# jerinphilip/whisper.tflite

Measured on AMD Instinct MI355X. Metric: audio-sec/s (RTF) whisper-tiny 30s clips batch=32 at 1/2/4/8 MI355X, higher is better.
Workload: dtype f32 (operands as two fp16 planes, f16 MFMA, f32 accumulate); 1 GPU; whisper-tiny batch=32x30s synthetic mel U(-1,1.5), fp32, random-init weights (BASELINE.json configs[1]); mel resident in HBM -> token ids on host; clips_per_gpu=32, global_batch=32, decoder_positions=30, argmax_steps=27, parallelism=clip-parallel dp1, one RCCL all_gather of id records per 8 batches, pipelined=True, batches_in_flight=10, decoder=2 consecutive steps' batches share one decoder chain (dec_pair, dec_group), last_batches_announced=2, priming_batches=1

## Files before the change

### include/wt_debug.h

```cpp
#ifndef WT_DEBUG_H_
#define WT_DEBUG_H_
#include "wt_capi.h"
#ifdef __cplusplus
extern "C" {
#endif
int wt_dbg_gemm(wt_engine* h, int M, int N, int K, const float* A, const float* W, const float* bias,
                const float* R, const float* pos, int pos_period, int epi, float* C);
int wt_dbg_gemm_planes(wt_engine* h, int M, int N, int K, const float* A, const float* W, const float* bias,
                       const float* R, const float* pos, int pos_period, int epi, int planes_out, int iters, float* C,
                       float* avg_ms, int n_cu );
int wt_dbg_set_forced_ids(wt_engine* h, const int64_t* ids, int clips);
int wt_dbg_set_plane_gemm_mode(int mode);
int wt_dbg_gemm_planes_ln(wt_engine* h, int M, int K, const float* A, const float* W, const float* bias, const float* R,
                          const float* pos, int pos_period, int epi, const float* ln_g, const float* ln_b, int n_cu,
                          float* C, float* ln_out, float* ln_y32, int* fused);
int wt_dbg_encoder_attention_planes(wt_engine* h, int batch, int T, int heads, const float* qkv, int iters, float* out,
                                    float* avg_ms);
int wt_dbg_gemm_bench(wt_engine* h, int M, int N, int K, int epi, int variant, int iters, float* avg_ms);
int wt_dbg_interference(wt_engine* h, const float* d_mel, int batch, int n_enc, int chain_len, int blocks,
                        float* enc_ms, float* chain_ms);
int wt_dbg_concurrency(wt_engine* h, const float* d_mel, int batch, int n_dec, int n_enc, float* dec_ms,
                       float* enc_ms);
int wt_dbg_dec_gemm_bench(wt_engine* h, int kind, int B, int N, int K, int rows, int iters, float* avg_us);
int wt_dbg_dec_gemm(wt_engine* h, int mode, int B, int N, int K, const float* X, const float* W,
                    const float* bias, const float* R, float* Y, int64_t* argmax_out);
int wt_dbg_dec_ln_gemm(wt_engine* h, int B, int N, int K, const float* xin, const int64_t* ids, int pos,
                       const float* tok_emb, const float* pos_emb, int n_vocab, int n_pos,
// ... 179 lines not shown
```

### whisper.tflite_amd/__init__.py

```python
from __future__ import annotations

import ctypes
import enum
import os
import types
from ctypes import (POINTER, byref, c_char_p, c_float, c_int, c_int32, c_int64, c_long, c_size_t,
                    c_uint64, c_void_p)

import numpy as np

_HERE = os.path.dirname(os.path.abspath(__file__))
LIB_PATH = os.environ.get("WT_LIB_PATH") or os.path.join(_HERE, "lib", "libwhisper-tflite.so")

WT_OK = 0
WT_MAX_IDS = 32
WT_PIPELINE_DEPTH = 24
WT_LANGUAGE_AUTO = -1
CHUNK_SAMPLES = 480000
STATUS_NAMES = {0: "WT_OK", 1: "WT_ERR_INVALID_ARG", 2: "WT_ERR_IO", 3: "WT_ERR_FORMAT",
                4: "WT_ERR_UNSUPPORTED", 5: "WT_ERR_DEVICE", 6: "WT_ERR_BUFFER"}

CAPI_SYMBOLS = [
    "wt_device_alloc", "wt_device_free", "wt_device_upload", "wt_device_download", "wt_device_synchronize",
    "wt_engine_create", "wt_engine_destroy", "wt_last_error", "wt_engine_dims",
# ... 4 lines not shown
    "wt_encdec_tokens_full_batch", "wt_encdec_tokens_full_batch_dev", "wt_transcribe_tokens_full_batch_dev",
    "wt_last_segments", "wt_last_segment_text", "wt_vocab_segments", "wt_vocab_seek_step", "wt_last_windows",
    "wt_transcribe_long_batch", "wt_last_file_text", "wt_last_window_files",
    "wt_vocab_split_words", "wt_vocab_merge_punctuation", "wt_dtw_path",
    "wt_engine_set_alignment_heads", "wt_last_words", "wt_last_word_text",
    "wt_last_scores", "wt_last_token_logprobs", "wt_last_segment_scores", "wt_last_decode_info", "wt_last_best_of",
    "wt_language_count", "wt_detect_language_batch", "wt_detect_language_batch_dev", "wt_detect_language_pcm", "wt_last_languages",
    "wt_last_timings", "wt_last_beam_scores", "wt_last_kernel_stats", "wt_decode_text", "wt_language_id", "wt_lang_code", "wt_wav_read_legacy",
    "wt_vocab_info", "wt_filters", "wt_write_synthetic_weights", "wt_write_synthetic_vocab",
    "wt_vocab_open", "wt_vocab_close", "wt_vocab_get_info", "wt_vocab_get_filters", "wt_vocab_size", "wt_vocab_token",
    "wt_vocab_decode", "wt_log_mel_spectrogram", "wt_convert_tflite", "wt_shutdown",
]
DEBUG_SYMBOLS = [
    "wt_dbg_cross_absorbed", "wt_dbg_cross_absorbed_bf16", "wt_dbg_gemm_planes_ln", "wt_dbg_gemm", "wt_dbg_gemm_bench", "wt_dbg_dec_gemm_bench", "wt_dbg_dec_gemm", "wt_dbg_dec_ln_gemm", "wt_dbg_layernorm", "wt_dbg_encoder_attention",
    "wt_dbg_cross_attention", "wt_dbg_self_attention", "wt_dbg_interference", "wt_dbg_concurrency",
    "wt_dbg_gemm_planes", "wt_dbg_set_plane_gemm_mode", "wt_dbg_set_forced_ids", "wt_dbg_dec_gemm_bf16", "wt_dbg_dec_ln_gemm_bf16",
    "wt_dbg_self_attention_bf16", "wt_dbg_cross_attention_bf16", "wt_dbg_encoder_attention_planes", "wt_dbg_gemm_bf16", "wt_dbg_gemm_bf16_ln", "wt_dbg_encoder_attention_bf16",
    "wt_dbg_beam_topk", "wt_dbg_beam_step", "wt_dbg_beam_reorder", "wt_dbg_beam_finalize",
    "wt_dbg_beam_full_step", "wt_dbg_beam_full_finalize",
    "wt_dbg_dec_gemm_ksplit", "wt_dbg_dec_ln_gemm_rows", "wt_dbg_dec_logits", "wt_dbg_select_token",
    "wt_dbg_cross_absorbed_chain", "wt_dbg_absorbed_query_matrix", "wt_dbg_language_head", "wt_dbg_self_attention_long",
    "wt_dbg_self_attention_prefill", "wt_dbg_self_attention_long_gather",
    "wt_dbg_self_attention_long_ragged", "wt_dbg_self_attention_prefill_ragged", "wt_dbg_dec_ln_gemm_ragged", "wt_dbg_ragged_cap",
    "wt_dbg_timestamp_select", "wt_dbg_token_scores", "wt_dbg_sample_select", "wt_dbg_suppress_logits",
    "wt_dbg_sample_select_group", "wt_dbg_best_of_begin", "wt_dbg_best_of_pick",
    "wt_dbg_frontend_dims", "wt_dbg_frontend_stages", "wt_dbg_log_clipmax", "wt_dbg_mel_normalize", "wt_dbg_mel_transpose",
    "wt_dbg_pcm_to_planes",
    "wt_dbg_gemm_addressed", "wt_dbg_plane_gemm_plan", "wt_dbg_gemm_ln_fused", "wt_dbg_layernorm_planes", "wt_dbg_f32_to_planes", "wt_dbg_encoder_attention_at",
    "wt_dbg_encoder_scales", "wt_dbg_f16_scale_for", "wt_dbg_gemm_planes_scaled",
    "wt_dbg_cross_attention_records", "wt_dbg_cross_attention_records_bf16", "wt_dbg_cross_combine", "wt_dbg_cross_combine_bf16",
    "wt_dbg_align_scores", "wt_dbg_align_matrix", "wt_dbg_align_dtw", "wt_dbg_last_alignment", "wt_dbg_set_alignment",
# ... 102 lines not shown
        L.wt_write_synthetic_weights.argtypes = [c_char_p, c_char_p, c_uint64]
        L.wt_write_synthetic_vocab.argtypes = [c_char_p, c_int]
        L.wt_vocab_open.argtypes = [c_char_p, c_int, POINTER(c_void_p)]
        L.wt_vocab_close.argtypes = [c_void_p]
        L.wt_vocab_close.restype = None
        L.wt_vocab_get_info.argtypes = [c_void_p, ip32]
        L.wt_vocab_get_filters.argtypes = [c_void_p, fp, c_size_t, ip32, ip32]
        L.wt_vocab_size.argtypes = [c_void_p]
        L.wt_vocab_token.argtypes = [c_void_p, c_int, c_char_p, c_size_t, POINTER(c_size_t)]
        L.wt_vocab_decode.argtypes = [c_void_p, ip64, c_int, c_int, c_char_p, c_size_t, POINTER(c_size_t)]
        L.wt_log_mel_spectrogram.argtypes = [fp, c_int, fp, c_int, c_int, c_int, fp, c_size_t, POINTER(c_int)]
        L.wt_convert_tflite.argtypes = [c_char_p, c_char_p]
        L.wt_dbg_gemm.argtypes = [c_void_p, c_int, c_int, c_int, fp, fp, fp, fp, fp, c_int, c_int, fp]
        L.wt_dbg_gemm_planes.argtypes = [c_void_p, c_int, c_int, c_int, fp, fp, fp, fp, fp, c_int, c_int, c_int, c_int, fp,
                                         POINTER(c_float), c_int]
        L.wt_dbg_encoder_attention_planes.argtypes = [c_void_p, c_int, c_int, c_int, fp, c_int, fp, POINTER(c_float)]
        L.wt_dbg_cross_absorbed.argtypes = [c_void_p, c_int, c_int, c_int, c_int, c_int, fp, fp, fp, fp, fp, c_int, POINTER(c_float)]
        L.wt_dbg_cross_absorbed_bf16.argtypes = L.wt_dbg_cross_absorbed.argtypes
        L.wt_dbg_cross_absorbed_chain.argtypes = [c_void_p, c_int, c_int, c_int, c_int, c_int, c_int, c_int, c_int, POINTER(fp),
                                                  fp, fp, fp, c_int, c_int, c_int, fp, fp]
        L.wt_dbg_absorbed_query_matrix.argtypes = [c_int, c_int, fp, fp, fp, fp, fp]
        L.wt_dbg_gemm_planes_ln.argtypes = [c_void_p, c_int, c_int, fp, fp, fp, fp, fp, c_int, c_int, fp, fp, c_int, fp, fp, fp,
                                            POINTER(c_int)]
        L.wt_dbg_gemm_bf16.argtypes = [c_void_p, c_int, c_int, c_int, fp, fp, fp, fp, fp, c_int, c_int, c_int, c_int, fp,
                                       POINTER(c_float)]
        L.wt_dbg_encoder_attention_bf16.argtypes = [c_void_p, c_int, c_int, c_int, fp, c_int, fp, POINTER(c_float)]
        L.wt_dbg_gemm_bf16_ln.argtypes = [c_void_p, c_int, c_int, c_int, fp, fp, fp, fp, fp, fp, fp, fp, fp, POINTER(c_int)]
        L.wt_dbg_gemm_bench.argtypes = [c_void_p, c_int, c_int, c_int, c_int, c_int, c_int, POINTER(c_float)]
        L.wt_dbg_dec_gemm_bench.argtypes = [c_void_p, c_int, c_int, c_int, c_int, c_int, c_int, POINTER(c_float)]
        L.wt_dbg_dec_gemm.argtypes = [c_void_p, c_int, c_int, c_int, c_int, fp, fp, fp, fp, fp, ip64]
# ... 719 lines not shown

    def dbg_gemm_planes(self, A, W, bias=None, R=None, pos=None, epi=1, planes_out=False, iters=0, n_cu=0):
        A, W = _f32(A), _f32(W)
        M, K = A.shape
        N = W.shape[0]
        C = np.zeros((M, N), np.float32)
        bias = _f32(bias) if bias is not None else np.zeros(N, np.float32)
        R = _f32(R) if R is not None else None
        pos = _f32(pos) if pos is not None else None
        ms = c_float(0)
        self._check(lib().wt_dbg_gemm_planes(self._h, M, N, K, _fp(A), _fp(W), _fp(bias), _fp(R), _fp(pos),
                                             pos.shape[0] if pos is not None else 0, epi, int(planes_out), iters, _fp(C),
                                             byref(ms), int(n_cu)))
        return (C, ms.value) if iters > 0 else C

    def dbg_gemm_planes_ln(self, A, W, bias, ln_g, ln_b, R=None, pos=None, epi=5, n_cu=0, want_y32=True):
        A, W = _f32(A), _f32(W)
        M, K = A.shape
        assert W.shape[0] == 384
        C = np.zeros((M, 384), np.float32)
        ln = np.zeros((M, 384), np.float32)
        y32 = np.zeros((M, 384), np.float32) if want_y32 else None
        R = _f32(R) if R is not None else None
        pos = _f32(pos) if pos is not None else None
        fused = ctypes.c_int(0)
        self._check(lib().wt_dbg_gemm_planes_ln(self._h, M, K, _fp(A), _fp(W), _fp(_f32(bias)), _fp(R), _fp(pos),
                                                pos.shape[0] if pos is not None else 0, epi, _fp(_f32(ln_g)), _fp(_f32(ln_b)),
                                                int(n_cu), _fp(C), _fp(ln), _fp(y32) if y32 is not None else None, byref(fused)))
        return C, ln, y32, bool(fused.value)

# ... 832 lines not shown
```

### whisper.tflite_amd/csrc/capi_debug.cpp

```cpp
#include "wt_debug.h"

#include <hip/hip_runtime.h>

#include <algorithm>
#include <array>
#include <cmath>
#include <cstdio>
#include <cstdlib>
#include <cstring>
#include <limits>
#include <memory>
#include <vector>

#include "capi_internal.h"
#include "kernels.h"

namespace {
template <class T>
struct DevArr {
  T* p = nullptr;
  size_t n = 0;
  explicit DevArr(size_t n_, const T* host = nullptr) : n(n_) {
    hipchk(hipMalloc(reinterpret_cast<void**>(&p), std::max<size_t>(n, 1) * sizeof(T)), "hipMalloc");
    if (host && n) hipchk(hipMemcpy(p, host, n * sizeof(T), hipMemcpyHostToDevice), "H2D");
// ... 197 lines not shown
int wt_dbg_gemm_planes(wt_engine* h, int M, int N, int K, const float* A, const float* W, const float* bias,
                       const float* R, const float* pos, int pos_period, int epi, int planes_out, int iters, float* C,
                       float* avg_ms, int n_cu) {
  if (!h || !A || !W || !C || N % 128 || K % 32 || M < 1 || n_cu < 0) return WT_ERR_INVALID_ARG;
  return guarded(h, [&] {
    const float sa = wt::f16_scale_for(max_abs(A, size_t(M) * K)), sw = wt::f16_scale_for(max_abs(W, size_t(N) * K));
    const DevPlanes dA(A, size_t(M) * K, sa);
    const DevArr<unsigned short> dW(weight_planes(W, N, K, sw));
    DevArr<float> dB(N, bias), dC(size_t(M) * N, R), dP(pos ? size_t(pos_period) * N : 0, pos);
    const float out_bound = max_abs(A, size_t(M) * K) * max_abs(W, size_t(N) * K) * float(K) + (bias ? max_abs(bias, N) : 0.0f);
    const float so = wt::f16_scale_for(out_bound);
    DevPlanes dO(nullptr, size_t(M) * N, 1.0f);
    wt::PlaneGemmArgs g;
    dense_gemm_args(g, M, N, K, dB.p, dC.p, dP.p, pos_period);
    g.A = dA.ptr(); g.a_plane = dA.plane; g.W = dW.p; g.a_scale = sa; g.w_scale = sw; g.n_cu = n_cu;
    if (planes_out) { g.P = dO.ptr(); g.p_plane = dO.plane; g.out_scale[0] = so; }
    hipStream_t st = h->impl->stream();
    wt::launch_gemm_planes(g, epi, st);
    h->impl->sync();
    if (planes_out) dO.to_host(C, size_t(M) * N, so); else dC.to_host(C, size_t(M) * N);
    if (avg_ms && iters > 0) *avg_ms = time_launches(st, 3, iters, [&] { wt::launch_gemm_planes(g, epi, st); });
  });
}

int wt_dbg_set_forced_ids(wt_engine* h, const int64_t* ids, int clips) {
  if (!h || clips < 0 || clips > 4096 || (clips && !ids)) return WT_ERR_INVALID_ARG;
  return guarded(h, [&] {
    h->impl->forced_ids.assign(ids, ids + size_t(clips) * 32);
    for (long long v : h->impl->forced_ids)
      if (v < 0) throw wt::Error(wt::kErrInvalidArg, "forced ids must be token ids");
  });
}

int wt_dbg_set_plane_gemm_mode(int mode) {
  if (mode < 0 || mode > 4) return WT_ERR_INVALID_ARG;
  wt::set_plane_gemm_mode(mode);
  return WT_OK;
}

int wt_dbg_gemm_planes_ln(wt_engine* h, int M, int K, const float* A, const float* W, const float* bias, const float* R,
                          const float* pos, int pos_period, int epi, const float* ln_g, const float* ln_b, int n_cu,
                          float* C, float* ln_out, float* ln_y32, int* fused) {
  const int N = 384;
  if (!h || !A || !W || !C || !ln_g || !ln_b || !ln_out || !fused || K % 32 || M < 1 || n_cu < 0) return WT_ERR_INVALID_ARG;
  return guarded(h, [&] {
    const float sa = wt::f16_scale_for(max_abs(A, size_t(M) * K)), sw = wt::f16_scale_for(max_abs(W, size_t(N) * K));
    const DevPlanes dA(A, size_t(M) * K, sa);
    const DevArr<unsigned short> dW(weight_planes(W, N, K, sw));
    DevArr<float> dB(N, bias), dC(size_t(M) * N, R), dP(pos ? size_t(pos_period) * N : 0, pos), dG(N, ln_g), dS(N, ln_b),
        dY(size_t(M) * N);
    DevArr<int> dF(1);
    hipStream_t st = h->impl->stream();
// ... 1441 lines not shown
    g.kv_batch = kv_batch; g.kv_heads = kv_heads; g.kv_dmodel = kv_dmodel;
    g.M = M; g.N = N; g.K = K; g.n_cu = n_cu;
    DevArr<float> dC(out_format == 0 ? size_t(c_len) : 0, static_cast<const float*>(out));
    DevArr<unsigned short> dO(out_format == 1 ? 2 * size_t(c_len) : out_format == 2 ? size_t(c_len) : 0,
                              static_cast<const unsigned short*>(out));
    if (out_format == 0) {
      g.C = dC.p + c_off; g.R = g.C;
    } else {
      g.P = dO.p + c_off; g.p_plane = c_len; g.seg = seg;
      if (out_format == 1) g.out_scale[0] = out_scale[0], g.out_scale[1] = out_scale[1], g.out_scale[2] = out_scale[2];
    }
    if (kind == 1) {
      const float sa = wt::f16_scale_for(max_abs(A, size_t(a_len))), sw = wt::f16_scale_for(max_abs(W, size_t(N) * K));
      const DevPlanes dA(A, size_t(a_len), sa);
      const DevArr<unsigned short> dW(weight_planes(W, N, K, sw));
      g.A = dA.ptr(); g.a_plane = dA.plane; g.W = dW.p; g.a_scale = sa; g.w_scale = sw;
      wt::launch_gemm_planes(g, epi, st);
      h->impl->sync();
    } else {
      const DevBf16 dA(A, size_t(a_len)), dW(W, size_t(N) * K);
      g.A = dA.ptr(); g.W = dW.ptr();
      wt::launch_gemm_bf16_planes(g, epi, st);
      h->impl->sync();
    }
    if (out_format == 0) dC.to_host(static_cast<float*>(out)); else dO.to_host(static_cast<unsigned short*>(out));
  });
}

int wt_dbg_plane_gemm_plan(int family, int M, int N, int K, int epi, int planes_out, int ln, int n_cu, int c_rpb, int ldc,
                           int32_t plan[4]) {
  if (!plan || family < 0 || family > 1 || M < 1 || N < 1 || K < 1 || n_cu < 0) return WT_ERR_INVALID_ARG;
// ... 106 lines not shown
                              int guard_rows, void* out) {
  const bool epi_ok = planes_out ? (epi == wt::kEpiBias || epi == (wt::kEpiBias | wt::kEpiGelu))
                                 : (epi == wt::kEpiBias || epi == (wt::kEpiBias | wt::kEpiGelu) || epi == (wt::kEpiBias | wt::kEpiResidual));
  if (!h || !A || !W || !bias || !out || !out_scale || !epi_ok || M < 1 || N < 128 || N % 128 || K < 32 || K % 32 || n_cu < 0 ||
      guard_rows < 0 || seg < 0) {
    return WT_ERR_INVALID_ARG;
  }
  return guarded(h, [&] {
    const size_t cells = size_t(M + guard_rows) * N;
    const DevPlanes dA(A, size_t(M) * K, a_scale);
    const DevArr<unsigned short> dW(weight_planes(W, N, K, w_scale));
    DevArr<float> dB(N, bias), dC(planes_out ? 0 : cells, static_cast<const float*>(out));
    DevArr<unsigned short> dO(planes_out ? 2 * cells : 0, static_cast<const unsigned short*>(out));
    wt::PlaneGemmArgs g;
    dense_gemm_args(g, M, N, K, dB.p, planes_out ? nullptr : dC.p, nullptr, 0);
    g.A = dA.ptr(); g.a_plane = dA.plane; g.W = dW.p; g.a_scale = a_scale; g.w_scale = w_scale; g.n_cu = n_cu;
    if (planes_out) {
      g.P = dO.p; g.p_plane = long(cells); g.seg = seg;
      g.out_scale[0] = out_scale[0]; g.out_scale[1] = out_scale[1]; g.out_scale[2] = out_scale[2];
    }
    wt::launch_gemm_planes(g, epi, h->impl->stream());
    h->impl->sync();
    if (planes_out) dO.to_host(static_cast<unsigned short*>(out)); else dC.to_host(static_cast<float*>(out));
  });
}

int wt_dbg_encoder_attention_at(wt_engine* h, int kind, int variant, int batch, int T, int heads, int guard_rows,
                                const float* qkv, const float scales[4], void* out) {
  if (!h || !qkv || !out || kind < 0 || kind > 2 || guard_rows < 0 || batch < 0 || T < 0 || heads < 0 || (kind == 1 && !scales)) {
    return WT_ERR_INVALID_ARG;
  }
// ... 143 lines not shown
```

### whisper.tflite_amd/csrc/engine.cpp

```cpp
#include "engine_internal.h"

#include <fcntl.h>
#include <sys/mman.h>
#include <sys/stat.h>
#include <unistd.h>

#include <chrono>
#include <cmath>
#include <complex>
#include <cstdio>
#include <cstdlib>
#include <cstring>
#include <stdexcept>

#include "kernels.h"

namespace wt {

namespace {
size_t round_up(size_t v, size_t m) { return (v + m - 1) / m * m; }
}


std::vector<unsigned short> tile_weights_f16(const float* W, int N, int K, float* scale) {
// ... 678 lines not shown
    const int prio = dp && dp[0] == 'l' ? prio_lo : prio_hi;
    for (auto& ds : dstream_) HIPCHK(hipStreamCreateWithPriority(&ds, hipStreamNonBlocking, prio));
  }
  pick_decoder_streams();
  for (auto& e : ev_) HIPCHK(hipEventCreate(&e));
  for (Slot& sl : slots_) {
    for (hipEvent_t* e : {&sl.enc_begin, &sl.enc_mid, &sl.enc_done, &sl.dec_begin, &sl.dec_done}) {
      HIPCHK(hipEventCreate(e));
    }
    sl.h_ids = pinned<long long>(4096 * 32);
    sl.h_n = pinned<int>(4096);
    sl.h_flag = pinned<int>(1);
    *sl.h_flag = 0;
    HIPCHK(hipMalloc(reinterpret_cast<void**>(&sl.d_flag), sizeof(int)));
  }
}

Engine::Engine(const std::string& model_prefix, const std::string& vocab_path, bool multilingual,
               int device_id, bool monolith, const std::string& weights_path)
    : device_(device_id), monolith_(monolith), multilingual_(multilingual) {
  read_vocab_file(vocab_path, multilingual, &filters_, &vocab_);
  if (monolith) language = 0;
  open_device();
  try {
    create_streams();
    upload_weights(weights_path.empty() ? model_prefix + ".wtw" : weights_path);
    if (vocab_.n_vocab != dims_.n_vocab && verbose) {
      std::fprintf(stderr, "[wt] note: vocab file n_vocab %d != model n_vocab %d\n", vocab_.n_vocab,
                   dims_.n_vocab);
    }
// ... 14 lines not shown
    build_frontend_tables();
  } catch (...) {
    release();
    throw;
  }
}

Engine::~Engine() { release(); }

void Engine::release() noexcept {
  (void)hipSetDevice(device_);
  for (hipStream_t st : {stream_full_, stream_masked_})
    if (st) (void)hipStreamSynchronize(st);
  for (auto& ds : dstream_)
    if (ds) (void)hipStreamSynchronize(ds);
  for (auto& g : graphs_) (void)hipGraphExecDestroy(g.second.exec);
  graphs_.clear();
  for (void* p : ws_.owned) (void)hipFree(p);
  ws_.owned.clear();
  for (void* p : allocations_) (void)hipFree(p);
  allocations_.clear();
  for (auto& e : ev_) {
    if (e) (void)hipEventDestroy(e);
    e = nullptr;
  }
  for (Slot& sl : slots_) {
    for (hipEvent_t* e : {&sl.enc_begin, &sl.enc_mid, &sl.enc_done, &sl.dec_begin, &sl.dec_done}) {
      if (*e) (void)hipEventDestroy(*e);
      *e = nullptr;
    }
// ... 405 lines not shown
    if (no_ln_fuse || !on_planes(consumer)) return;
    e.g.ln_g = gain; e.g.ln_b = shift; e.g.ln_P = lnp; e.g.ln_plane = ln_plane; e.g.ln_scale = a_scale(consumer);
  };
  auto enc_gemm = [&](const EncGemm& e) {
    const EncLinear& w = *e.w;
    const double flops = 2.0 * e.g.M * w.N * double(w.k);
    if (on_planes(w)) {
      PlaneGemmArgs g = e.g;
      g.W = bf ? w.wbf : w.wp; g.bias = w.bias; g.N = w.N; g.K = bf ? w.kbf : w.kp;
      if (e.to_planes) {
        g.P = e.P; g.p_plane = e.p_plane; g.seg = e.seg;
        for (int i = 0; e.out_scale && i < (e.seg ? 3 : 1); ++i) g.out_scale[i] = e.out_scale[i];
      } else {
        g.C = e.C32;
      }
      if (!bf) g.n_cu = cus, g.a_scale = w.sc.a, g.w_scale = w.sc.w;
      kt_begin(kKcGemm, flops, 0);
      ln_done = bf ? launch_gemm_bf16_planes(g, e.epi, stream_) : launch_gemm_planes(g, e.epi, stream_);
      kt_end();
      return PlaneOperand{g.P, g.p_plane};
    }
    GemmArgs g;
    g.A = e.A32; g.W = w.w32; g.C = e.C32; g.bias = w.bias; g.R = e.g.R; g.pos = e.g.pos;
    g.M = e.g.M; g.N = w.N; g.K = w.k32;
    g.a_rpb = e.g.a_rpb; g.a_bs = e.g.a_bs; g.lda = e.g.lda; g.c_rpb = e.g.c_rpb; g.c_bs = e.g.c_bs; g.ldc = e.g.ldc;
    g.pos_period = e.g.pos_period; g.kv_batch = e.g.kv_batch; g.kv_heads = e.g.kv_heads; g.kv_dmodel = e.g.kv_dmodel;
    g.variant = alt; g.a_scale = w.sc.a; g.w_scale = w.sc.w;
    kt_begin(kKcGemmAlt, flops, 0);
    launch_gemm(g, e.epi, stream_);
    kt_end();
    if (!e.to_planes) return PlaneOperand{nullptr, 0};
// ... 1039 lines not shown
```

### whisper.tflite_amd/csrc/engine.h

```cpp
#pragma once
#include <hip/hip_runtime.h>

#include <algorithm>
#include <array>
#include <cstdint>
#include <functional>
#include <map>
#include <stdexcept>
#include <string>
#include <utility>
#include <vector>

#include "decode_results.h"
#include "error.h"
#include "host_util.h"
#include "wtw_format.h"

namespace wt {

struct TsPart;
struct TsState;

struct BeamPart;
struct BeamFullPart;
// ... 322 lines not shown
  int ragged_stride() const { return 2 * full_cap() + 2; }
  void ensure_ragged_workspace();
  struct AlignWorkspace {
    float *W = nullptr, *stats = nullptr, *C = nullptr;
    size_t w_elems = 0, c_elems = 0, s_elems = 0;
    unsigned char* trace = nullptr;
    int *jump = nullptr, *lfn = nullptr;
    int *h_jump = nullptr, *h_lfn = nullptr;
  } aw_;
  static constexpr size_t kAlignWeightBytes = size_t(256) << 20;
  static constexpr long long kFullKey = -1000;
  static constexpr long long kBeamFullKey = -2000;
  static constexpr long long kBestOfKey = -3000;

  int enc_cus_masked_ = 0;
 public:
  int pipelined_encoder_cus() const { return enc_cus_masked_ > 0 ? enc_cus_masked_ : n_cu_; }
 private:
  int device_ = 0, n_cu_ = 0, reserve_ = 0;
  bool monolith_ = false, multilingual_ = true;
  hipStream_t stream_ = nullptr;
  hipStream_t stream_full_ = nullptr, stream_masked_ = nullptr;
  hipEvent_t ev_switch_ = nullptr;
  void select_stream(bool pipelined);
  void pick_decoder_streams();
  void encode_enqueue(const float* d_mel, int batch);
  static constexpr int kDecStreams = 8, kSlots = 24;
  int n_dec_streams_ = 3;
  hipStream_t dstream_[kDecStreams] = {};
  static constexpr int kEncAsDec = kDecStreams;
  hipStream_t dec_stream_at(int i) const { return i == kEncAsDec ? (stream_masked_ ? stream_masked_ : stream_full_) : dstream_[i]; }
  hipEvent_t ev_[2] = {nullptr, nullptr};
// ... 165 lines not shown
```

### whisper.tflite_amd/csrc/k_gemm_planes.hip

```cpp
#include <hip/hip_runtime.h>

#include <algorithm>
#include <cstdlib>
#include <cstring>

#include "bf16_split.h"
#include "kernels.h"

namespace wt {

static int g_plane_gemm_mode = -1;
int plane_gemm_mode() {
  if (g_plane_gemm_mode < 0) {
    const char* v = getenv("WT_PLANE_GEMM_MODE");
    g_plane_gemm_mode = v ? atoi(v) : 2;
  }
  return g_plane_gemm_mode;
}
void set_plane_gemm_mode(int m) { g_plane_gemm_mode = m; }

namespace {

using f32x16 = __attribute__((ext_vector_type(16))) float;
using f32x4 = __attribute__((ext_vector_type(4))) float;
using half8 = __attribute__((ext_vector_type(8))) _Float16;
using half4 = __attribute__((ext_vector_type(4))) _Float16;
using u32x4 = __attribute__((ext_vector_type(4))) unsigned;

constexpr int BK = 32;

struct PlaneGemmDev {
  const _Float16* A;
  long a_plane;
  const _Float16* W;
// ... 580 lines not shown
    dma.issue(1, 1);
    dma_done_but<T::QPW>();
  } else {
    dma_done();
  }
  phase_end();
  if (w.wm == 1) phase_end();
  f.load_first(smem);
  reads_done();
  phase_end();
  pingpong_k_loop<0>(smem, dma, f, acc, nkt, w.wm, st);
  planes_epilogue<EPI, PLANES_OUT, T::WN, LN>(g, acc, smem, dma.m0, dma.n0, w.wid, w.wm, w.wn, w.lane);
  st.store(w.lane, w.wid);
}

template <int EPI>
__global__ __launch_bounds__(512, 2) void gemm_planes_pp16_persist(PlaneGemmDev g, int total_tiles) {
  using T = PlaneTile<4, 3, 3>;
  constexpr bool PLANES_OUT = true;
  static_assert((EPI & ~(kEpiBias | kEpiGelu)) == 0, "bias / GELU epilogues with plane output");
  constexpr int P = 1;
  constexpr int kEpiStores = T::MI * T::NI * 4;
  PpStamps st;
  extern __shared__ __attribute__((aligned(16))) unsigned char smem[];
  const int grid = gridDim.x;
  const WavePos w = wave_pos<T>();
  int vid = blockIdx.x;
  StageDma<T> dma(g, smem, w.wid, total_tiles, vid, w.lane);
  Acc16<T::MI, T::NI> acc;
  Frag16<T> f(w.wm, w.wn, w.lane);

  const int nkt = g.K / BK;
  dma.issue(0, stage_of<P>(0));
  dma.issue(1, stage_of<P>(1));
  dma_done_but<T::QPW>();
  phase_end();
  for (;;) {
    if (w.wm == 1) phase_end();
    acc.zero();
    f.load_first(smem + stage_of<P>(0) * T::kStage);
    reads_done();
    phase_end();
    pingpong_k_loop<P>(smem, dma, f, acc, nkt, w.wm, st);
    const int m_cur = dma.m0, n_cur = dma.n0;
    const int next = vid + grid;
    const bool has_next = next < total_tiles;
    const bool whole = m_cur + T::BM <= g.M;
    auto prefetch = [&]() {
      if (has_next) {
        dma.set_tile(g, total_tiles, next, w.lane);
        dma.issue(0, stage_of<P>(0));
      }
    };
    planes_epilogue<EPI, PLANES_OUT, T::WN, false>(g, acc, smem, m_cur, n_cur, w.wid, w.wm, w.wn, w.lane,
                                                   ActiveEpilogueHook<decltype(prefetch)>{prefetch});
    if (!has_next) break;
    if (whole) {
      dma_done_but<kEpiStores>();
    } else {
      dma_done();
    }
    phase_end();
    dma.issue(1, stage_of<P>(1));
    vid = next;
  }
}

template <int EPI, bool PLANES_OUT, int WN, int NI, int MI = 3, bool LN = false>
void launch_planes_shape(const PlaneGemmDev& g, hipStream_t s, const PlaneGemmPlan& plan, int n_cu = 0) {
  using T = PlaneTile<WN, NI, MI>;
  const int blocks = ((g.M + T::BM - 1) / T::BM) * (g.N / T::BN);
  constexpr size_t smem = 2 * T::kStage;
  static const bool raised = [] {
    (void)hipFuncSetAttribute(reinterpret_cast<const void*>(&gemm_planes_tile<EPI, PLANES_OUT, WN, NI, MI, LN>),
                              hipFuncAttributeMaxDynamicSharedMemorySize, 160 * 1024);
    return true;
  }();
  (void)raised;
  if constexpr (WN == 4 && NI == 3 && MI == 3) {
    if constexpr (PLANES_OUT && !LN && (EPI & ~(kEpiBias | kEpiGelu)) == 0) {
      if (plan.schedule == 3) {
        const int cu = n_cu > 0 ? n_cu : 256;
        static const bool raised_p = [] {
          (void)hipFuncSetAttribute(reinterpret_cast<const void*>(&gemm_planes_pp16_persist<EPI>), hipFuncAttributeMaxDynamicSharedMemorySize,
                                    160 * 1024);
          return true;
        }();
        (void)raised_p;
        WT_LAUNCH_TIMED((gemm_planes_pp16_persist<EPI>), dim3(cu), dim3(512), smem, s, g, blocks);
        return;
      }
    }
    if (plan.schedule == 2) {
      static const bool raised_pp16 = [] {
        (void)hipFuncSetAttribute(reinterpret_cast<const void*>(&gemm_planes_pp16<EPI, PLANES_OUT, LN>),
                                  hipFuncAttributeMaxDynamicSharedMemorySize, 160 * 1024);
        return true;
      }();
      (void)raised_pp16;
      WT_LAUNCH_TIMED((gemm_planes_pp16<EPI, PLANES_OUT, LN>), dim3(blocks), dim3(512), smem, s, g);
      return;
    }
    if (plan.schedule == 1) {
      static const bool raised_pp = [] {
// ... 3 lines not shown
      }();
      (void)raised_pp;
      WT_LAUNCH_TIMED((gemm_planes_pp<EPI, PLANES_OUT, MI, LN>), dim3(blocks), dim3(512), smem, s, g);
      return;
    }
  }
  if (plan.schedule != 0) throw Error(kErrUnsupported, "plane GEMM: the plan names a schedule this tile does not have");
  WT_LAUNCH_TIMED((gemm_planes_tile<EPI, PLANES_OUT, WN, NI, MI, LN>), dim3(blocks), dim3(128 * WN), smem, s, g);
}

constexpr bool ln_fusable(int epi, bool planes_out) {
  return !planes_out && (epi == (kEpiBias | kEpiResidual) || epi == (kEpiBias | kEpiGelu | kEpiPos));
}

template <int EPI, bool PLANES_OUT>
bool launch_planes(const PlaneGemmDev& g, int n_cu, hipStream_t s) {
  const PlaneGemmPlan plan = plane_gemm_plan(g.M, g.N, g.K, EPI, PLANES_OUT, g.ln_P != nullptr, n_cu, plane_gemm_mode());
  if constexpr (ln_fusable(EPI, PLANES_OUT)) {
    if (plan.fused) {
      if (plan.tile == 2) {
        launch_planes_shape<EPI, false, 4, 3, 4, true>(g, s, plan);
      } else {
        launch_planes_shape<EPI, false, 4, 3, 3, true>(g, s, plan);
      }
      return true;
    }
  }
  if (plan.fused) throw Error(kErrUnsupported, "plane GEMM: the plan fuses a LayerNorm this epilogue cannot");
  if (plan.tile == 2) {
    launch_planes_shape<EPI, PLANES_OUT, 4, 3, 4>(g, s, plan);
  } else if (plan.tile == 1) {
    launch_planes_shape<EPI, PLANES_OUT, 4, 3, 3>(g, s, plan, n_cu);
  } else {
    launch_planes_shape<EPI, PLANES_OUT, 2, 2, 3>(g, s, plan);
  }
  return false;
}

}

std::vector<unsigned short> split_weight_planes(const float* W, int N, int K, int Kpad, float scale) {
  if (N % 16 != 0 || Kpad % 32 != 0 || K > Kpad) throw Error(kErrInvalidArg, "split_weight_planes: N % 16, Kpad % 32");
  std::vector<unsigned short> out(size_t(2) * N * Kpad, 0);
  const int nkt = Kpad / 32;
  for (int n = 0; n < N; ++n) {
    const int rg = n / 16, r = n % 16;
    for (int k = 0; k < K; ++k) {
      const float v = W[size_t(n) * K + k] * scale;
      const _Float16 h = static_cast<_Float16>(v);
      const _Float16 l = static_cast<_Float16>(v - static_cast<float>(h));
      const int kt = k / 32, c = (k % 32) / 8, e = k % 8;
      const size_t blk = (size_t(rg) * nkt + kt) * 2 * 512;
      const size_t at = size_t(r * 4 + (c ^ chunk_swizzle(r))) * 8 + e;
      std::memcpy(out.data() + blk + at, &h, 2);
      std::memcpy(out.data() + blk + 512 + at, &l, 2);
    }
  }
  return out;
}

PlaneGemmPlan plane_gemm_plan(int M, int N, int K, int epi, bool planes_out, bool ln, int n_cu, int mode) {
  static const int forced = [] {
    const char* v = getenv("WT_PLANE_TILE");
    return v ? atoi(v) : 0;
  }();
  const int cu = n_cu > 0 ? n_cu : 256;
  auto rounds = [&](long tiles) { return (tiles + cu - 1) / cu; };
  const long rt192 = (M + 191) / 192, rt256 = (M + 255) / 256;
  const bool can_wide = N % 384 == 0;
  const double c_wide = can_wide ? 192.0 * 3 * rounds(rt192 * (N / 384)) : 1e30;
  const double c_tall = can_wide ? 256.0 * 3 * 1.08 * rounds(rt256 * (N / 384)) : 1e30;
  const double c_narrow = 192.0 * 1.1 * rounds(rt192 * (N / 128));
  int pick = c_wide <= c_narrow ? (c_tall < c_wide ? 2 : 1) : (c_tall < c_narrow ? 2 : 0);
  if (forced == 128) pick = 0;
  if (forced == 384 && can_wide) pick = 1;
  if (forced == 256 && can_wide) pick = 2;
  PlaneGemmPlan p;
  p.tile = pick;
  p.fused = ln_fusable(epi, planes_out) && ln && N == 384 && pick != 0;
  if (pick == 1) {
    const long blocks = rt192 * (N / 384);
    const bool persist = planes_out && !p.fused && (epi & ~(kEpiBias | kEpiGelu)) == 0 && mode == 2 && cu % 8 == 0 &&
                         blocks >= 2 * cu && (K / BK) % 2 == 0 && K / BK >= 4;
    p.schedule = persist ? 3 : (mode == 2 || mode == 4) ? 2 : mode == 1 ? 1 : 0;
  }
  return p;
}

bool launch_gemm_planes(const PlaneGemmArgs& a, int epi, hipStream_t s) {
  PlaneGemmDev g{};
  g.A = reinterpret_cast<const _Float16*>(a.A); g.a_plane = a.a_plane;
  g.W = reinterpret_cast<const _Float16*>(a.W);
  g.C = a.C; g.P = reinterpret_cast<_Float16*>(a.P); g.p_plane = a.p_plane;
  g.bias = a.bias; g.R = a.R; g.pos = a.pos;
  g.M = a.M; g.N = a.N; g.K = a.K;
  g.a_rpb = a.a_rpb; g.a_bs = a.a_bs; g.lda = a.lda;
  g.c_rpb = a.c_rpb; g.c_bs = a.c_bs; g.ldc = a.ldc;
  g.pos_period = a.pos_period;
  g.kv_batch = a.kv_batch; g.kv_heads = a.kv_heads; g.kv_dmodel = a.kv_dmodel;
// ... 6 lines not shown
    throw Error(kErrInvalidArg, "plane GEMM LayerNorm fusion: needs gain and shift, fp32 output, contiguous [M][N] rows");
  }
  const bool planes = a.P != nullptr;
  if (a.N % 128 != 0 || a.K % BK != 0 || a.M < 1 || a.c_rpb < 32 || a.pos_period < (epi & kEpiPos ? 32 : 1) || a.lda % 8 != 0 ||
      a.a_bs % 8 != 0 || a.ldc % 8 != 0 || a.c_bs % 8 != 0 || (planes && (g.seg % 8 != 0 || (a.N + g.seg - 1) / g.seg > 3)) ||
      (!planes && !a.C) || !(a.a_scale > 0.0f) || !(a.w_scale > 0.0f)) {
    throw Error(kErrInvalidArg, "plane GEMM shape outside the kernel contract");
  }
  {
    const long a_span = a.a_plane + (long)((a.M - 1) / a.a_rpb) * a.a_bs + (long)std::min(a.a_rpb, a.M) * a.lda + a.K + 64;
    if (a.a_plane < 0 || a.a_bs < 0 || 2 * a_span >= (1L << 32)) {
      throw Error(kErrInvalidArg, "plane GEMM operand spans more than the 4 GiB its 32-bit offsets reach");
    }
  }
  switch (epi | (planes ? 256 : 0)) {
    case kEpiBias: return launch_planes<kEpiBias, false>(g, a.n_cu, s);
    case kEpiBias | kEpiGelu: return launch_planes<kEpiBias | kEpiGelu, false>(g, a.n_cu, s);
    case kEpiBias | kEpiResidual: return launch_planes<kEpiBias | kEpiResidual, false>(g, a.n_cu, s);
    case kEpiBias | kEpiGelu | kEpiPos: return launch_planes<kEpiBias | kEpiGelu | kEpiPos, false>(g, a.n_cu, s);
    case kEpiBias | kEpiKvLayout: return launch_planes<kEpiBias | kEpiKvLayout, false>(g, a.n_cu, s);
    case kEpiBias | kEpiPower: return launch_planes<kEpiBias | kEpiPower, false>(g, a.n_cu, s);
    case kEpiBias | 256: return launch_planes<kEpiBias, true>(g, a.n_cu, s);
    case kEpiBias | kEpiGelu | 256: return launch_planes<kEpiBias | kEpiGelu, true>(g, a.n_cu, s);
    default: throw Error(kErrInvalidArg, "unsupported plane GEMM epilogue combination");
  }
}

}
```

### whisper.tflite_amd/csrc/kernels.h

```cpp
#pragma once
#include <hip/hip_runtime.h>
#include <hip/hip_ext.h>

#include <cstdint>
#include <vector>

#include "error.h"

namespace wt {

struct LaunchTimer {
  hipEvent_t start = nullptr, stop = nullptr;
};
extern thread_local LaunchTimer g_launch_timer;

#define WT_LAUNCH_TIMED(kernel, grid, block, smem, stream, ...)                                                      \
  do {                                                                                                                \
    if (::wt::g_launch_timer.start) {                                                                                 \
      hipExtLaunchKernelGGL(kernel, grid, block, smem, stream, ::wt::g_launch_timer.start, ::wt::g_launch_timer.stop, \
                            0, __VA_ARGS__);                                                                          \
    } else {                                                                                                          \
      hipLaunchKernelGGL(kernel, grid, block, smem, stream, __VA_ARGS__);                                             \
    }                                                                                                                 \
  } while (0)
// ... 48 lines not shown
  int c_rpb = 1 << 30;
  long c_bs = 0;
  int ldc = 0;
  int pos_period = 1;
  int kv_batch = 0, kv_heads = 0, kv_dmodel = 0;
  float a_scale = 1.0f, w_scale = 1.0f;
  float out_scale[3] = {1.0f, 1.0f, 1.0f};
  int seg = 0;
  int n_cu = 256;
  const float *ln_g = nullptr, *ln_b = nullptr;
  unsigned short* ln_P = nullptr;
  long ln_plane = 0;
  float ln_scale = 1.0f;
  float* ln_y32 = nullptr;
  int* nonfinite = nullptr;
};
bool launch_gemm_planes(const PlaneGemmArgs& a, int epi, hipStream_t s);
int plane_gemm_mode();
void set_plane_gemm_mode(int m);
struct PlaneGemmPlan {
  int tile = 0, schedule = 0;
  bool fused = false;
};
PlaneGemmPlan plane_gemm_plan(int M, int N, int K, int epi, bool planes_out, bool ln, int n_cu, int mode);
bool launch_gemm_bf16_planes(const PlaneGemmArgs& a, int epi, hipStream_t s);
struct Bf16GemmPlan {
  int bm = 192, bn = 128;
  bool whole_row = false;
};
Bf16GemmPlan bf16_gemm_plan(int M, int N, int epi, bool bf16_out, bool ln, int c_rpb, int ldc);
std::vector<unsigned short> round_weights_bf16(const float* W, int N, int K, int Kpad);
std::vector<unsigned short> split_weight_planes(const float* W, int N, int K, int Kpad, float scale);

enum DecPro : int {
  kProNone = 0,
  kProLn = 1,
  kProCombine = 2
};
enum DecEpi : int {
// ... 392 lines not shown
```

Before: 152,200 audio-sec/s.

## Add per-XCD atomic tile claiming to persistent plane GEMM

Replaces the static stride scheduling (vid += grid) of the persistent pp16 plane GEMM with dynamic tile claiming. Each block draws its next tile from one of eight per-XCD atomic counters, and the last claimant resets the counter for the next launch. The intent is to balance uneven block progress when the encoder GEMM shares CUs with concurrent decoder work. It costs an atomic per tile, an extra LDS word and tail, and depends on the counter being left at zero between launches. Compile-gated timestamp instrumentation and debug hooks are also added.

```diff
diff --git a/include/wt_debug.h b/include/wt_debug.h
--- a/include/wt_debug.h
+++ b/include/wt_debug.h
@@ -11,6 +11,8 @@
                        float* avg_ms, int n_cu );
 int wt_dbg_set_forced_ids(wt_engine* h, const int64_t* ids, int clips);
 int wt_dbg_set_plane_gemm_mode(int mode);
+int wt_dbg_set_plane_tile(int tile);
+int wt_dbg_plane_claim_counters(wt_engine* h, int32_t counters[8]);
 int wt_dbg_gemm_planes_ln(wt_engine* h, int M, int K, const float* A, const float* W, const float* bias, const float* R,
                           const float* pos, int pos_period, int epi, const float* ln_g, const float* ln_b, int n_cu,
                           float* C, float* ln_out, float* ln_y32, int* fused);
diff --git a/whisper.tflite_amd/__init__.py b/whisper.tflite_amd/__init__.py
--- a/whisper.tflite_amd/__init__.py
+++ b/whisper.tflite_amd/__init__.py
@@ -42,7 +42,7 @@
 DEBUG_SYMBOLS = [
     "wt_dbg_cross_absorbed", "wt_dbg_cross_absorbed_bf16", "wt_dbg_gemm_planes_ln", "wt_dbg_gemm", "wt_dbg_gemm_bench", "wt_dbg_dec_gemm_bench", "wt_dbg_dec_gemm", "wt_dbg_dec_ln_gemm", "wt_dbg_layernorm", "wt_dbg_encoder_attention",
     "wt_dbg_cross_attention", "wt_dbg_self_attention", "wt_dbg_interference", "wt_dbg_concurrency",
-    "wt_dbg_gemm_planes", "wt_dbg_set_plane_gemm_mode", "wt_dbg_set_forced_ids", "wt_dbg_dec_gemm_bf16", "wt_dbg_dec_ln_gemm_bf16",
+    "wt_dbg_gemm_planes", "wt_dbg_set_plane_gemm_mode", "wt_dbg_plane_claim_counters", "wt_dbg_set_plane_tile", "wt_dbg_set_forced_ids", "wt_dbg_dec_gemm_bf16", "wt_dbg_dec_ln_gemm_bf16",
     "wt_dbg_self_attention_bf16", "wt_dbg_cross_attention_bf16", "wt_dbg_encoder_attention_planes", "wt_dbg_gemm_bf16", "wt_dbg_gemm_bf16_ln", "wt_dbg_encoder_attention_bf16",
     "wt_dbg_beam_topk", "wt_dbg_beam_step", "wt_dbg_beam_reorder", "wt_dbg_beam_finalize",
     "wt_dbg_beam_full_step", "wt_dbg_beam_full_finalize",
@@ -175,6 +175,8 @@
         L.wt_dbg_gemm.argtypes = [c_void_p, c_int, c_int, c_int, fp, fp, fp, fp, fp, c_int, c_int, fp]
         L.wt_dbg_gemm_planes.argtypes = [c_void_p, c_int, c_int, c_int, fp, fp, fp, fp, fp, c_int, c_int, c_int, c_int, fp,
                                          POINTER(c_float), c_int]
+        if hasattr(L, "wt_dbg_plane_claim_counters"):
+            L.wt_dbg_plane_claim_counters.argtypes = [c_void_p, ip32]
         L.wt_dbg_encoder_attention_planes.argtypes = [c_void_p, c_int, c_int, c_int, fp, c_int, fp, POINTER(c_float)]
         L.wt_dbg_cross_absorbed.argtypes = [c_void_p, c_int, c_int, c_int, c_int, c_int, fp, fp, fp, fp, fp, c_int, POINTER(c_float)]
         L.wt_dbg_cross_absorbed_bf16.argtypes = L.wt_dbg_cross_absorbed.argtypes
@@ -924,6 +926,11 @@
                                              byref(ms), int(n_cu)))
         return (C, ms.value) if iters > 0 else C
 
+    def dbg_plane_claim_counters(self):
+        out = (c_int32 * 8)()
+        self._check(lib().wt_dbg_plane_claim_counters(self._h, out))
+        return list(out)
+
     def dbg_gemm_planes_ln(self, A, W, bias, ln_g, ln_b, R=None, pos=None, epi=5, n_cu=0, want_y32=True):
         A, W = _f32(A), _f32(W)
         M, K = A.shape
diff --git a/whisper.tflite_amd/csrc/capi_debug.cpp b/whisper.tflite_amd/csrc/capi_debug.cpp
--- a/whisper.tflite_amd/csrc/capi_debug.cpp
+++ b/whisper.tflite_amd/csrc/capi_debug.cpp
@@ -235,6 +235,7 @@
     wt::PlaneGemmArgs g;
     dense_gemm_args(g, M, N, K, dB.p, dC.p, dP.p, pos_period);
     g.A = dA.ptr(); g.a_plane = dA.plane; g.W = dW.p; g.a_scale = sa; g.w_scale = sw; g.n_cu = n_cu;
+    g.claim = h->impl->plane_claim();
     if (planes_out) { g.P = dO.ptr(); g.p_plane = dO.plane; g.out_scale[0] = so; }
     hipStream_t st = h->impl->stream();
     wt::launch_gemm_planes(g, epi, st);
@@ -254,9 +255,25 @@
 }
 
 int wt_dbg_set_plane_gemm_mode(int mode) {
-  if (mode < 0 || mode > 4) return WT_ERR_INVALID_ARG;
+  if (mode < 0 || mode > 6) return WT_ERR_INVALID_ARG;
   wt::set_plane_gemm_mode(mode);
   return WT_OK;
+}
+
+int wt_dbg_set_plane_tile(int tile) {
+  if (tile != 0 && tile != 128 && tile != 256 && tile != 384) return WT_ERR_INVALID_ARG;
+  wt::set_plane_tile(tile);
+  return WT_OK;
+}
+
+int wt_dbg_plane_claim_counters(wt_engine* h, int32_t counters[8]) {
+  if (!h || !counters) return WT_ERR_INVALID_ARG;
+  return guarded(h, [&] {
+    h->impl->sync();
+    int32_t all[wt::kPlaneClaimWords];
+    hipchk(hipMemcpy(all, h->impl->plane_claim(), sizeof(all), hipMemcpyDeviceToHost), "D2H");
+    for (int x = 0; x < 8; ++x) counters[x] = all[x * wt::kPlaneClaimStride];
+  });
 }
 
 int wt_dbg_gemm_planes_ln(wt_engine* h, int M, int K, const float* A, const float* W, const float* bias, const float* R,
@@ -1728,7 +1745,7 @@
       const float sa = wt::f16_scale_for(max_abs(A, size_t(a_len))), sw = wt::f16_scale_for(max_abs(W, size_t(N) * K));
       const DevPlanes dA(A, size_t(a_len), sa);
       const DevArr<unsigned short> dW(weight_planes(W, N, K, sw));
-      g.A = dA.ptr(); g.a_plane = dA.plane; g.W = dW.p; g.a_scale = sa; g.w_scale = sw;
+      g.A = dA.ptr(); g.a_plane = dA.plane; g.W = dW.p; g.a_scale = sa; g.w_scale = sw; g.claim = h->impl->plane_claim();
       wt::launch_gemm_planes(g, epi, st);
       h->impl->sync();
     } else {
@@ -1865,7 +1882,7 @@
     DevArr<unsigned short> dO(planes_out ? 2 * cells : 0, static_cast<const unsigned short*>(out));
     wt::PlaneGemmArgs g;
     dense_gemm_args(g, M, N, K, dB.p, planes_out ? nullptr : dC.p, nullptr, 0);
-    g.A = dA.ptr(); g.a_plane = dA.plane; g.W = dW.p; g.a_scale = a_scale; g.w_scale = w_scale; g.n_cu = n_cu;
+    g.A = dA.ptr(); g.a_plane = dA.plane; g.W = dW.p; g.a_scale = a_scale; g.w_scale = w_scale; g.n_cu = n_cu; g.claim = h->impl->plane_claim();
     if (planes_out) {
       g.P = dO.p; g.p_plane = long(cells); g.seg = seg;
       g.out_scale[0] = out_scale[0]; g.out_scale[1] = out_scale[1]; g.out_scale[2] = out_scale[2];
diff --git a/whisper.tflite_amd/csrc/engine.cpp b/whisper.tflite_amd/csrc/engine.cpp
--- a/whisper.tflite_amd/csrc/engine.cpp
+++ b/whisper.tflite_amd/csrc/engine.cpp
@@ -716,6 +716,8 @@
     *sl.h_flag = 0;
     HIPCHK(hipMalloc(reinterpret_cast<void**>(&sl.d_flag), sizeof(int)));
   }
+  plane_claim_ = static_cast<int*>(dev_zeroed_bytes(kPlaneClaimWords * sizeof(int)));
+  HIPCHK(hipDeviceSynchronize());
 }
 
 Engine::Engine(const std::string& model_prefix, const std::string& vocab_path, bool multilingual,
@@ -760,6 +762,8 @@
     if (st) (void)hipStreamSynchronize(st);
   for (auto& ds : dstream_)
     if (ds) (void)hipStreamSynchronize(ds);
+  persist_stamps_dump();
+  plane_claim_ = nullptr;
   for (auto& g : graphs_) (void)hipGraphExecDestroy(g.second.exec);
   graphs_.clear();
   for (void* p : ws_.owned) (void)hipFree(p);
@@ -1195,7 +1199,7 @@
       } else {
         g.C = e.C32;
       }
-      if (!bf) g.n_cu = cus, g.a_scale = w.sc.a, g.w_scale = w.sc.w;
+      if (!bf) g.n_cu = cus, g.a_scale = w.sc.a, g.w_scale = w.sc.w, g.claim = plane_claim_;
       kt_begin(kKcGemm, flops, 0);
       ln_done = bf ? launch_gemm_bf16_planes(g, e.epi, stream_) : launch_gemm_planes(g, e.epi, stream_);
       kt_end();
diff --git a/whisper.tflite_amd/csrc/engine.h b/whisper.tflite_amd/csrc/engine.h
--- a/whisper.tflite_amd/csrc/engine.h
+++ b/whisper.tflite_amd/csrc/engine.h
@@ -360,8 +360,10 @@
   static constexpr long long kBestOfKey = -3000;
 
   int enc_cus_masked_ = 0;
+  int* plane_claim_ = nullptr;
  public:
   int pipelined_encoder_cus() const { return enc_cus_masked_ > 0 ? enc_cus_masked_ : n_cu_; }
+  int* plane_claim() const { return plane_claim_; }
  private:
   int device_ = 0, n_cu_ = 0, reserve_ = 0;
   bool monolith_ = false, multilingual_ = true;
diff --git a/whisper.tflite_amd/csrc/k_gemm_planes.hip b/whisper.tflite_amd/csrc/k_gemm_planes.hip
--- a/whisper.tflite_amd/csrc/k_gemm_planes.hip
+++ b/whisper.tflite_amd/csrc/k_gemm_planes.hip
@@ -1,14 +1,17 @@
 #include <hip/hip_runtime.h>
 
 #include <algorithm>
+#include <cstdio>
 #include <cstdlib>
 #include <cstring>
+#include <string>
 
 #include "bf16_split.h"
 #include "kernels.h"
 
 namespace wt {
 
+constexpr bool kPlaneClaimDefault = true;
 static int g_plane_gemm_mode = -1;
 int plane_gemm_mode() {
   if (g_plane_gemm_mode < 0) {
@@ -18,6 +21,8 @@
   return g_plane_gemm_mode;
 }
 void set_plane_gemm_mode(int m) { g_plane_gemm_mode = m; }
+static int g_plane_tile_forced = -1;
+void set_plane_tile(int rows_or_cols) { g_plane_tile_forced = rows_or_cols; }
 
 namespace {
 
@@ -628,8 +633,47 @@
   st.store(w.lane, w.wid);
 }
 
+
+#ifdef WT_PERSIST_STAMPS
+constexpr int kPsRing = 512, kPsBlocks = 256, kPsWords = 16, kPsTiles = 8;
+__device__ long long g_ps_rec[kPsBlocks * kPsRing * kPsWords];
+__device__ int g_ps_launches[kPsBlocks];
+#endif
+constexpr int kPersistTail = 256;
+struct PersistStamps {
+#ifdef WT_PERSIST_STAMPS
+  long long* t;
+  int* id;
+  int n = 0;
+  bool on;
+  __device__ __forceinline__ PersistStamps(long long* t_, int* id_, bool on_) : t(t_), id(id_), on(on_) {
+    if (on) t[0] = (long long)__builtin_amdgcn_s_memrealtime();
+  }
+  __device__ __forceinline__ void tile_done(int vid) {
+    if (on && n < kPsTiles) t[1 + n] = (long long)__builtin_amdgcn_s_memrealtime(), id[n] = vid;
+    ++n;
+  }
+  __device__ __forceinline__ void store(int grid, int total, bool claimed) {
+    if (!on || blockIdx.x >= kPsBlocks) return;
+    const int slot = g_ps_launches[blockIdx.x];
+    g_ps_launches[blockIdx.x] = slot + 1;
+    long long* r = g_ps_rec + ((size_t)blockIdx.x * kPsRing + slot % kPsRing) * kPsWords;
+    r[0] = t[0];
+    r[1] = (long long)__builtin_amdgcn_s_memrealtime();
+    r[2] = (long long)grid | ((long long)total << 32);
+    r[3] = (long long)n | ((long long)(claimed ? 1 : 0) << 32);
+    for (int i = 0; i < kPsTiles; ++i) r[4 + i] = i < n ? t[1 + i] : 0;
+    for (int i = 0; i < kPsTiles / 2; ++i)
+      r[12 + i] = (long long)(unsigned)(2 * i < n ? id[2 * i] : -1) | ((long long)(2 * i + 1 < n ? id[2 * i + 1] : -1) << 32);
+  }
+#else
+  __device__ __forceinline__ void tile_done(int) {}
+  __device__ __forceinline__ void store(int, int, bool) {}
+#endif
+};
+
 template <int EPI>
-__global__ __launch_bounds__(512, 2) void gemm_planes_pp16_persist(PlaneGemmDev g, int total_tiles) {
+__global__ __launch_bounds__(512, 2) void gemm_planes_pp16_persist(PlaneGemmDev g, int total_tiles, int* claim) {
   using T = PlaneTile<4, 3, 3>;
   constexpr bool PLANES_OUT = true;
   static_assert((EPI & ~(kEpiBias | kEpiGelu)) == 0, "bias / GELU epilogues with plane output");
@@ -637,9 +681,22 @@
   constexpr int kEpiStores = T::MI * T::NI * 4;
   PpStamps st;
   extern __shared__ __attribute__((aligned(16))) unsigned char smem[];
+  int& claim_word = *reinterpret_cast<int*>(smem + 2 * T::kStage);
   const int grid = gridDim.x;
   const WavePos w = wave_pos<T>();
+#ifdef WT_PERSIST_STAMPS
+  static_assert(16 + 8 * (1 + kPsTiles) + 4 * kPsTiles <= kPersistTail, "the stamps fit behind the stages");
+  PersistStamps ps(reinterpret_cast<long long*>(smem + 2 * T::kStage + 16), reinterpret_cast<int*>(smem + 2 * T::kStage + 16 + 8 * (1 + kPsTiles)),
+                   w.wid == 0 && w.lane == 0);
+#else
+  PersistStamps ps;
+#endif
   int vid = blockIdx.x;
+  const int xcd = vid & 7;
+  const bool claimed = claim != nullptr;
+  const bool drawer = claimed && w.wid == 0;
+  int* const counter = claim + xcd * kPlaneClaimStride;
+  int draw = 0;
   StageDma<T> dma(g, smem, w.wid, total_tiles, vid, w.lane);
   Acc16<T::MI, T::NI> acc;
   Frag16<T> f(w.wm, w.wn, w.lane);
@@ -652,15 +709,24 @@
   for (;;) {
     if (w.wm == 1) phase_end();
     acc.zero();
+    if (drawer && w.lane == 0) draw = __hip_atomic_fetch_add(counter, 1, __ATOMIC_RELAXED, __HIP_MEMORY_SCOPE_AGENT);
     f.load_first(smem + stage_of<P>(0) * T::kStage);
     reads_done();
     phase_end();
     pingpong_k_loop<P>(smem, dma, f, acc, nkt, w.wm, st);
+    if (drawer && w.lane == 0) {
+      *reinterpret_cast<volatile int*>(&claim_word) = draw;
+      if (draw == ((total_tiles - xcd + 7) >> 3) - 1) __hip_atomic_store(counter, 0, __ATOMIC_RELAXED, __HIP_MEMORY_SCOPE_AGENT);
+    }
     const int m_cur = dma.m0, n_cur = dma.n0;
-    const int next = vid + grid;
-    const bool has_next = next < total_tiles;
+    int next = vid + grid;
+    bool has_next = next < total_tiles;
     const bool whole = m_cur + T::BM <= g.M;
     auto prefetch = [&]() {
+      if (claimed) {
+        next = xcd + 8 * ((grid >> 3) + __builtin_amdgcn_readfirstlane(*reinterpret_cast<volatile int*>(&claim_word)));
+        has_next = next < total_tiles;
+      }
       if (has_next) {
         dma.set_tile(g, total_tiles, next, w.lane);
         dma.issue(0, stage_of<P>(0));
@@ -668,6 +734,7 @@
     };
     planes_epilogue<EPI, PLANES_OUT, T::WN, false>(g, acc, smem, m_cur, n_cur, w.wid, w.wm, w.wn, w.lane,
                                                    ActiveEpilogueHook<decltype(prefetch)>{prefetch});
+    ps.tile_done(vid);
     if (!has_next) break;
     if (whole) {
       dma_done_but<kEpiStores>();
@@ -678,10 +745,11 @@
     dma.issue(1, stage_of<P>(1));
     vid = next;
   }
+  ps.store(grid, total_tiles, claimed);
 }
 
 template <int EPI, bool PLANES_OUT, int WN, int NI, int MI = 3, bool LN = false>
-void launch_planes_shape(const PlaneGemmDev& g, hipStream_t s, const PlaneGemmPlan& plan, int n_cu = 0) {
+void launch_planes_shape(const PlaneGemmDev& g, hipStream_t s, const PlaneGemmPlan& plan, int n_cu = 0, int* claim = nullptr) {
   using T = PlaneTile<WN, NI, MI>;
   const int blocks = ((g.M + T::BM - 1) / T::BM) * (g.N / T::BN);
   constexpr size_t smem = 2 * T::kStage;
@@ -701,7 +769,7 @@
           return true;
         }();
         (void)raised_p;
-        WT_LAUNCH_TIMED((gemm_planes_pp16_persist<EPI>), dim3(cu), dim3(512), smem, s, g, blocks);
+        WT_LAUNCH_TIMED((gemm_planes_pp16_persist<EPI>), dim3(cu), dim3(512), smem + kPersistTail, s, g, blocks, plan.claim ? claim : nullptr);
         return;
       }
     }
@@ -735,7 +803,7 @@
 }
 
 template <int EPI, bool PLANES_OUT>
-bool launch_planes(const PlaneGemmDev& g, int n_cu, hipStream_t s) {
+bool launch_planes(const PlaneGemmDev& g, int n_cu, int* claim, hipStream_t s) {
   const PlaneGemmPlan plan = plane_gemm_plan(g.M, g.N, g.K, EPI, PLANES_OUT, g.ln_P != nullptr, n_cu, plane_gemm_mode());
   if constexpr (ln_fusable(EPI, PLANES_OUT)) {
     if (plan.fused) {
@@ -751,7 +819,7 @@
   if (plan.tile == 2) {
     launch_planes_shape<EPI, PLANES_OUT, 4, 3, 4>(g, s, plan);
   } else if (plan.tile == 1) {
-    launch_planes_shape<EPI, PLANES_OUT, 4, 3, 3>(g, s, plan, n_cu);
+    launch_planes_shape<EPI, PLANES_OUT, 4, 3, 3>(g, s, plan, n_cu, claim);
   } else {
     launch_planes_shape<EPI, PLANES_OUT, 2, 2, 3>(g, s, plan);
   }
@@ -780,11 +848,35 @@
   return out;
 }
 
+void persist_stamps_dump() {
+#ifdef WT_PERSIST_STAMPS
+  static int n_dumps = 0;
+  const char* out = getenv("WT_PERSIST_STAMPS_OUT");
+  if (!out) return;
+  std::vector<int> launches(kPsBlocks);
+  if (hipMemcpyFromSymbol(launches.data(), HIP_SYMBOL(g_ps_launches), sizeof(int) * kPsBlocks) != hipSuccess) return;
+  if (*std::max_element(launches.begin(), launches.end()) == 0) return;
+  std::vector<long long> rec(size_t(kPsBlocks) * kPsRing * kPsWords);
+  if (hipMemcpyFromSymbol(rec.data(), HIP_SYMBOL(g_ps_rec), sizeof(long long) * rec.size()) != hipSuccess) return;
+  const std::string path = std::string(out) + "." + std::to_string(n_dumps++);
+  if (FILE* fp = fopen(path.c_str(), "wb")) {
+    const int head[4] = {kPsBlocks, kPsRing, kPsWords, kPsTiles};
+    fwrite(head, sizeof(int), 4, fp);
+    fwrite(launches.data(), sizeof(int), kPsBlocks, fp);
+    fwrite(rec.data(), sizeof(long long), rec.size(), fp);
+    fclose(fp);
+  }
+  std::fill(launches.begin(), launches.end(), 0);
+  (void)hipMemcpyToSymbol(HIP_SYMBOL(g_ps_launches), launches.data(), sizeof(int) * kPsBlocks);
+#endif
+}
+
 PlaneGemmPlan plane_gemm_plan(int M, int N, int K, int epi, bool planes_out, bool ln, int n_cu, int mode) {
-  static const int forced = [] {
+  if (g_plane_tile_forced < 0) {
     const char* v = getenv("WT_PLANE_TILE");
-    return v ? atoi(v) : 0;
-  }();
+    g_plane_tile_forced = v ? std::max(atoi(v), 0) : 0;
+  }
+  const int forced = g_plane_tile_forced;
   const int cu = n_cu > 0 ? n_cu : 256;
   auto rounds = [&](long tiles) { return (tiles + cu - 1) / cu; };
   const long rt192 = (M + 191) / 192, rt256 = (M + 255) / 256;
@@ -801,9 +893,11 @@
   p.fused = ln_fusable(epi, planes_out) && ln && N == 384 && pick != 0;
   if (pick == 1) {
     const long blocks = rt192 * (N / 384);
-    const bool persist = planes_out && !p.fused && (epi & ~(kEpiBias | kEpiGelu)) == 0 && mode == 2 && cu % 8 == 0 &&
+    const bool pp16 = mode == 2 || mode == 4 || mode == 5 || mode == 6;
+    const bool persist = planes_out && !p.fused && (epi & ~(kEpiBias | kEpiGelu)) == 0 && pp16 && mode != 4 && cu % 8 == 0 &&
                          blocks >= 2 * cu && (K / BK) % 2 == 0 && K / BK >= 4;
-    p.schedule = persist ? 3 : (mode == 2 || mode == 4) ? 2 : mode == 1 ? 1 : 0;
+    p.schedule = persist ? 3 : pp16 ? 2 : mode == 1 ? 1 : 0;
+    p.claim = persist && (mode == 6 || (mode == 2 && kPlaneClaimDefault));
   }
   return p;
 }
@@ -840,14 +934,14 @@
     }
   }
   switch (epi | (planes ? 256 : 0)) {
-    case kEpiBias: return launch_planes<kEpiBias, false>(g, a.n_cu, s);
-    case kEpiBias | kEpiGelu: return launch_planes<kEpiBias | kEpiGelu, false>(g, a.n_cu, s);
-    case kEpiBias | kEpiResidual: return launch_planes<kEpiBias | kEpiResidual, false>(g, a.n_cu, s);
-    case kEpiBias | kEpiGelu | kEpiPos: return launch_planes<kEpiBias | kEpiGelu | kEpiPos, false>(g, a.n_cu, s);
-    case kEpiBias | kEpiKvLayout: return launch_planes<kEpiBias | kEpiKvLayout, false>(g, a.n_cu, s);
-    case kEpiBias | kEpiPower: return launch_planes<kEpiBias | kEpiPower, false>(g, a.n_cu, s);
-    case kEpiBias | 256: return launch_planes<kEpiBias, true>(g, a.n_cu, s);
-    case kEpiBias | kEpiGelu | 256: return launch_planes<kEpiBias | kEpiGelu, true>(g, a.n_cu, s);
+    case kEpiBias: return launch_planes<kEpiBias, false>(g, a.n_cu, a.claim, s);
+    case kEpiBias | kEpiGelu: return launch_planes<kEpiBias | kEpiGelu, false>(g, a.n_cu, a.claim, s);
+    case kEpiBias | kEpiResidual: return launch_planes<kEpiBias | kEpiResidual, false>(g, a.n_cu, a.claim, s);
+    case kEpiBias | kEpiGelu | kEpiPos: return launch_planes<kEpiBias | kEpiGelu | kEpiPos, false>(g, a.n_cu, a.claim, s);
+    case kEpiBias | kEpiKvLayout: return launch_planes<kEpiBias | kEpiKvLayout, false>(g, a.n_cu, a.claim, s);
+    case kEpiBias | kEpiPower: return launch_planes<kEpiBias | kEpiPower, false>(g, a.n_cu, a.claim, s);
+    case kEpiBias | 256: return launch_planes<kEpiBias, true>(g, a.n_cu, a.claim, s);
+    case kEpiBias | kEpiGelu | 256: return launch_planes<kEpiBias | kEpiGelu, true>(g, a.n_cu, a.claim, s);
     default: throw Error(kErrInvalidArg, "unsupported plane GEMM epilogue combination");
   }
 }
diff --git a/whisper.tflite_amd/csrc/kernels.h b/whisper.tflite_amd/csrc/kernels.h
--- a/whisper.tflite_amd/csrc/kernels.h
+++ b/whisper.tflite_amd/csrc/kernels.h
@@ -86,15 +86,21 @@
   float ln_scale = 1.0f;
   float* ln_y32 = nullptr;
   int* nonfinite = nullptr;
-};
+  int* claim = nullptr;
+};
+constexpr int kPlaneClaimStride = 32;
+constexpr int kPlaneClaimWords = 8 * kPlaneClaimStride;
 bool launch_gemm_planes(const PlaneGemmArgs& a, int epi, hipStream_t s);
 int plane_gemm_mode();
 void set_plane_gemm_mode(int m);
+void set_plane_tile(int tile);
 struct PlaneGemmPlan {
   int tile = 0, schedule = 0;
   bool fused = false;
+  bool claim = false;
 };
 PlaneGemmPlan plane_gemm_plan(int M, int N, int K, int epi, bool planes_out, bool ln, int n_cu, int mode);
+void persist_stamps_dump();
 bool launch_gemm_bf16_planes(const PlaneGemmArgs& a, int epi, hipStream_t s);
 struct Bf16GemmPlan {
   int bm = 192, bn = 128;
```

After: 151,400 audio-sec/s. Within noise of the previous version (-0.5%).
